# levayz/diffusion_finetuning

Measured on AMD Instinct MI355X. Metric: images/s SD1.5 LoRA rank-4 512^2 train step, higher is better.
Workload: dtype f16; 1 GPU; SD1.5 UNet-only LoRA rank=4, batch=4/GPU, 512^2 (64x64x4 latents), f16 storage/compute, fp32 accumulate + fp32 master LoRA, full train step (fwd+bwd+clip+AdamW); global_batch=4, parallelism=dp1, lora_params=1246464, overflow=False, hipgraph=True, conv_autotune=True, rccl_ranks=1

## Files before the change

diffusion_finetuning_amd/_native.py:

```python
import ctypes
import os
import threading

import torch

_LIB_PATH = os.environ.get("DFA_LIB_PATH") or os.path.join(os.path.dirname(os.path.abspath(__file__)), "lib", "liblora_hip.so")
_lib = None
_lock = threading.Lock()

ABI_VERSION = 9
PROF_KINDS = 18

_DTYPE_CODE = {torch.float32: 0, torch.float16: 1, torch.bfloat16: 2}

_vp, _i64, _i32, _f32 = ctypes.c_void_p, ctypes.c_int64, ctypes.c_int, ctypes.c_float


class GradProblem(ctypes.Structure):
    _fields_ = [
        ("S", _vp), ("P", _vp), ("out", _vp * 4),
        ("s_stride", _i64), ("p_stride", _i64), ("part_stride", _i64), ("M", _i64),
        ("C", _i32), ("r", _i32), ("rg", _i32), ("out_kn", _i32), ("n_blocks", _i32),
        ("scale", _f32),
    ]
# ... 76 lines not shown
                                            ctypes.c_uint64, _i32, _vp]),
    "ddpm_sample_step_keep_shared": (_i32, [_vp] * 11 + [_i32, _i64, _i64, _i32, _i32, _f32, _i32, _vp]),
    "ddpm_sample_multistep_keep_shared": (_i32, [_vp] * 13 + [_i32, _i64, _i64, _i32, _i32, _f32, _i32, _vp]),
    "ddpm_sample_sigma_init": (_i32, [_vp] * 7 + [_i32, _i64, _i32, _i32, _f32, _f32, _f32, _i32, _i32, ctypes.c_uint64, _i32, _vp]),
    "ddpm_sample_sigma": (_i32, [_vp] * 14 + [_i32, _i64, _i64, _i32, _i32, _i32, _f32, _i32, _vp]),
    "embed_rows_fwd": (_i32, [_vp, _vp, _vp, _i64, _i32, _i64, _i32, _vp]),
    "embed_rows_bwd": (_i32, [_vp, _vp, _vp, _vp, _i64, _i32, _i64, _i32, _i32, _vp]),
    "lora_adamw_rows": (_i32, [_vp, _vp, _vp, _vp, _vp, _i64, _i32, _vp, _f32, _f32, _f32, _f32, _f32, _f32, _f32, _i32, _vp]),
    "ti_rows_grad": (_i32, [_vp, _vp, _i64, _i32, _vp, _i32, _vp, _i32, _i32, _vp]),
    "ti_rows_adamw_decay": (_i32, [_vp, _i64, _i32, _vp, _i32, _vp, _vp, _vp, _f32, _f32, _f32, _f32, _f32, _f32, _i32, _f32, _f32,
                                   _vp]),
    "geglu_linear_bwd": (_i32, [_vp, _vp, _vp, _vp, _vp, _i64, _i32, _i32, _i32, _vp]),
    "geglu_gate_fwd": (_i32, [_vp, _vp, _i64, _i32, _i32, _vp]),
    "geglu_gate_bwd": (_i32, [_vp, _vp, _vp, _i64, _i32, _i32, _vp]),
    "attn_split_heads": (_i32, [_vp, _vp, _i32, _i32, _i32, _i32, _i32, _i32, _vp]),
    "attn_merge_heads": (_i32, [_vp, _vp, _i32, _i32, _i32, _i32, _i32, _i32, _vp]),
    "attn_merge_heads_strided": (_i32, [_vp, _vp, _i32, _i32, _i32, _i32, _i32, _i64, _i64, _i64, _i32, _vp]),
    "group_norm_act_workspace_bytes": (_i64, [_i32, _i32, _i32, _i32, _i32, _i32]),
    "group_norm_act_plan": (_i32, [_i32, _i32, _i32, _i32, _i32, _i32]),
    "group_norm_act_fwd": (_i32, [_vp] * 8 + [_i32, _i32, _i32, _i32, _f32, _i32, _i32, _i32, _vp]),
    "group_norm_act_bwd": (_i32, [_vp] * 10 + [_i32, _i32, _i32, _i32, _i32, _i32, _i32, _vp]),
    "group_norm_act_bwd_res": (_i32, [_vp] * 11 + [_i32, _i32, _i32, _i32, _i32, _i32, _vp]),
    "residual_bias_add_supported": (_i32, [_i32, _i32, _i32, _i32]),
    "residual_bias_add": (_i32, [_vp] * 5 + [_i32, _i32, _i32, _i32, _vp]),
    "tokens_nchw_supported": (_i32, [_i32, _i32, _i32, _i32]),
    "tokens_to_nchw_add": (_i32, [_vp] * 3 + [_i32, _i32, _i32, _i32, _vp]),
    "nchw_to_tokens": (_i32, [_vp] * 2 + [_i32, _i32, _i32, _i32, _vp]),
    "conv3x3_small_supported": (_i32, [_i32, _i32, _i32, _i32, _i32, _i32]),
    "conv3x3_small_workspace_bytes": (_i64, [_i32, _i32, _i32, _i32, _i32, _i32]),
    "conv3x3_small_plan": (_i32, [_i64, _i32, _i32, _i32]),
    "conv3x3_small_plan_channels": (_i32, [_i32, _i32, _i32]),
    "conv3x3_small_pack": (_i32, [_vp, _vp, _i32, _i32, _i32, _i32, _vp]),
    "conv3x3_small": (_i32, [_vp] * 5 + [_i64, _i32, _i32, _i32, _i32, _i32, _i32, _vp]),
    "add_layer_norm_max_channels": (_i32, []),
    "add_layer_norm_fwd": (_i32, [_vp] * 8 + [_i64, _i32, _f32, _i32, _vp]),
    "add_layer_norm_bwd": (_i32, [_vp] * 7 + [_i64, _i32, _i32, _vp]),
    "attn_ctx_supported": (_i32, [_i32, _i32, _i32, _i32, _i32, _i32]),
    "attn_ctx_fwd": (_i32, [_vp, _vp, _vp, _vp, _i32, _i32, _i32, _i32, _i32, _f32, _i32, _vp]),
    "attn_ctx_bwd_workspace_bytes": (_i64, [_i32, _i32, _i32, _i32, _i32]),
    "attn_ctx_fwd_strided": (_i32, [_vp, _vp, _vp, _vp, _i64, _i32, _i32, _i32, _i32, _i32, _f32, _i32, _vp]),
    "attn_ctx_bwd_strided": (_i32, [_vp] * 8 + [_i64, _i64, _i32, _i32, _i32, _i32, _i32, _f32, _i32, _vp]),
    "attn_flash_fwd_strided": (_i32, [_vp, _vp, _vp, _vp, _vp, _i64, _i32, _i32, _i32, _i32, _i32, _f32, _i32, _vp]),
    "attn_flash_bwd_strided": (_i32, [_vp] * 10 + [_i64, _i64, _i32, _i32, _i32, _i32, _i32, _f32, _i32, _vp]),
    "attn_ctx_bwd": (_i32, [_vp, _vp, _vp, _vp, _vp, _vp, _vp, _vp, _i32, _i32, _i32, _i32, _i32, _f32, _i32, _vp]),
    "attn_causal_supported": (_i32, [_i32, _i32, _i32, _i32, _i32]),
    "attn_causal_fwd_strided": (_i32, [_vp, _vp, _vp, _vp, _i64, _i32, _i32, _i32, _i32, _f32, _i32, _vp]),
    "attn_causal_bwd_workspace_bytes": (_i64, [_i32, _i32, _i32, _i32]),
    "attn_causal_bwd_strided": (_i32, [_vp] * 8 + [_i64, _i64, _i32, _i32, _i32, _i32, _f32, _i32, _vp]),
    "attn_flash_supported": (_i32, [_i32, _i32, _i32, _i32, _i32, _i32]),
    "attn_flash_fwd": (_i32, [_vp, _vp, _vp, _vp, _vp, _i32, _i32, _i32, _i32, _i32, _f32, _i32, _vp]),
    "attn_flash_bwd_workspace_bytes": (_i64, [_i32, _i32, _i32]),
    "attn_flash_bwd": (_i32, [_vp] * 10 + [_i32, _i32, _i32, _i32, _i32, _f32, _i32, _vp]),
    "attn_f32_supported": (_i32, [_i32, _i32, _i32, _i32, _i32]),
    "attn_f32_fwd": (_i32, [_vp, _vp, _vp, _vp, _vp, _i32, _i32, _i32, _i32, _i32, _f32, _vp]),
    "attn_f32_bwd_workspace_bytes": (_i64, [_i32, _i32, _i32]),
    "attn_f32_bwd": (_i32, [_vp] * 10 + [_i32, _i32, _i32, _i32, _i32, _f32, _vp]),
    "lora_distill_workspace_bytes": (_i64, [_i64, _i64]),
    "lora_distill_start": (_i32, [_vp, _i32, _i64, _i32, _i64, _vp, _vp]),
    "lora_distill_diff": (_i32, [_vp, _i32, _i64, _i32, _i32, _vp, _vp]),
    "lora_distill_rayleigh_ritz": (_i32, [_vp, _i32, _i32, _i32, ctypes.c_double, _i32, _vp, _vp]),
    "lora_distill_finalize": (_i32, [_vp, _i32, _i32, _f32, _i32, _vp, _vp, _vp]),
    "lora_quantile_clamp": (_i32, [_vp, _i64, _f32, _vp, _vp]),
    "lora_distill_wide_width": (_i32, [_i32]),
    "lora_distill_wide_workspace_bytes": (_i64, [_i64, _i64, _i32]),
    "lora_distill_wide_start": (_i32, [_vp, _i32, _i64, _i32, _i64, _vp, _vp]),
    "lora_distill_wide_diff": (_i32, [_vp, _i32, _i64, _i32, _i32, _i32, _vp, _vp]),
# ... 1112 lines not shown
def conv3x3_small_supported(N: int, Cin: int, Cout: int, H: int, W: int, dtype) -> bool:
    return dtype in (torch.float16, torch.bfloat16) and bool(lib().conv3x3_small_supported(N, Cin, Cout, H, W, dtype_code(dtype)))


def conv3x3_small_plan(pixels: int, Cin: int, Cout: int, dtype) -> bool:
    return dtype in (torch.float16, torch.bfloat16) and bool(lib().conv3x3_small_plan(int(pixels), Cin, Cout, dtype_code(dtype)))


def conv3x3_small_plan_channels(Cin: int, Cout: int, dtype) -> bool:
    return dtype in (torch.float16, torch.bfloat16) and bool(lib().conv3x3_small_plan_channels(Cin, Cout, dtype_code(dtype)))


def conv3x3_small_pack(weight, backward: bool):
    _require_device(weight)
    Cout, Cin = weight.shape[:2]
    packed = torch.empty(weight.numel(), dtype=weight.dtype, device=weight.device)
    _check(lib().conv3x3_small_pack(_ptr(weight), _ptr(packed), Cin, Cout, int(backward), dtype_code(weight.dtype),
                                    _stream(weight)), "conv3x3_small_pack")
    return packed


def conv3x3_small(x, pack, bias, Cout: int):
    _require_device(x, pack, bias)
    N, Cin, H, W = x.shape
    code = dtype_code(x.dtype)
    nbytes = int(lib().conv3x3_small_workspace_bytes(N, Cin, Cout, H, W, code))
    ws = torch.empty(max(nbytes, 16) // 4, dtype=torch.float32, device=x.device)
    y = torch.empty((N, Cout, H, W), dtype=x.dtype, device=x.device)
    _check(lib().conv3x3_small(_ptr(x), _ptr(pack), _ptr(bias), _ptr(y), _ptr(ws), nbytes, N, Cin, Cout, H, W, code, _stream(x)),
           "conv3x3_small")
    return y


def tokens_nchw_supported(N: int, C: int, HW: int, dtype) -> bool:
    return dtype in (torch.float16, torch.bfloat16) and bool(lib().tokens_nchw_supported(N, C, HW, dtype_code(dtype)))


def tokens_to_nchw_add(tok, res, shape):
    _require_device(tok, res)
    N, C, H, W = shape
    out = torch.empty(shape, dtype=tok.dtype, device=tok.device)
    _check(lib().tokens_to_nchw_add(_ptr(tok), _ptr(res), _ptr(out), N, C, H * W, dtype_code(tok.dtype), _stream(tok)),
           "tokens_to_nchw_add")
    return out


def nchw_to_tokens(x):
    _require_device(x)
    N, C, H, W = x.shape
    tok = torch.empty((N, H * W, C), dtype=x.dtype, device=x.device)
    _check(lib().nchw_to_tokens(_ptr(x), _ptr(tok), N, C, H * W, dtype_code(x.dtype), _stream(x)), "nchw_to_tokens")
    return tok


def add_layer_norm_supported(x) -> bool:
    C = x.shape[-1] if x.dim() else 0
    return (x.numel() > 0 and x.is_contiguous() and C % 8 == 0 and C <= lib().add_layer_norm_max_channels() and
            x.data_ptr() % 16 == 0)


def add_layer_norm_fwd(x, delta, gamma, beta, eps: float):
    _require_device(x, delta, gamma, beta)
    C = x.shape[-1]
    M = x.numel() // C
    h = None if delta is None else torch.empty_like(x)
    y = torch.empty_like(x)
# ... 262 lines not shown
```

diffusion_finetuning_amd/build_native.py:

```python
import hashlib
import os
import subprocess
import sys
from concurrent.futures import ThreadPoolExecutor

PKG_DIR = os.path.dirname(os.path.abspath(__file__))
CSRC = os.path.join(PKG_DIR, "csrc")
LIB_DIR = os.path.join(PKG_DIR, "lib")
LIB_PATH = os.path.join(LIB_DIR, "liblora_hip.so")
SOURCES = ["lora_gemm.hip", "lora_grad.hip", "ddpm_loss.hip", "optim.hip", "sandwich.hip", "norm.hip", "trunk_edges.hip", "conv_small.hip", "layer_norm.hip", "attn_ctx.hip", "attn_causal.hip", "attn_flash.hip", "attn_f32.hip", "embed.hip", "distill.hip", "distill_wide.hip", "prof.hip"]
HIPCC = os.environ.get("HIPCC", "/opt/rocm/bin/hipcc")
FLAGS = ["--offload-arch=gfx950", "-O3", "-std=c++17", "-fPIC", "-Wall", "-Wno-unused-function"]
SOURCE_FLAGS = {}


def _digest() -> str:
    h = hashlib.sha256()
    for name in sorted(os.listdir(CSRC)) + [os.path.join("..", "..", "include", "lora_hip.h")]:
        with open(os.path.join(CSRC, name), "rb") as f:
            h.update(name.encode())
            h.update(f.read())
    h.update(" ".join(FLAGS).encode())
    for name in sorted(SOURCE_FLAGS):
        h.update((name + " " + " ".join(SOURCE_FLAGS[name])).encode())
    return h.hexdigest()


def build(force: bool = False, verbose: bool = True, variant: str = "", defines=()) -> str:
    os.makedirs(LIB_DIR, exist_ok=True)
    lib_path = os.path.join(LIB_DIR, f"liblora_hip_{variant}.so") if variant else LIB_PATH
    obj_dir = os.path.join(LIB_DIR, f"obj_{variant}") if variant else LIB_DIR
    os.makedirs(obj_dir, exist_ok=True)
    stamp = os.path.join(LIB_DIR, f"liblora_hip_{variant}.stamp" if variant else "liblora_hip.stamp")
    digest = _digest() + (" " + " ".join(defines) if defines else "")
    if not force and os.path.exists(lib_path) and os.path.exists(stamp):
        with open(stamp) as f:
            if f.read().strip() == digest:
                return lib_path

    def compile_one(src: str) -> str:
        obj = os.path.join(obj_dir, src.replace(".hip", ".o"))
        cmd = [HIPCC, *FLAGS, *SOURCE_FLAGS.get(src, []), *defines, "-c", os.path.join(CSRC, src), "-o", obj]
        if verbose:
# ... 24 lines not shown
```

diffusion_finetuning_amd/conv.py:

```python
import torch
import torch.nn as nn
import torch.nn.functional as F
from torch.autograd.function import once_differentiable
from torch.utils.weak import WeakIdKeyDictionary

from . import _native as nat

ROUTES = ("auto", "hip", "stock")

_packs = WeakIdKeyDictionary()


def _key(weight):
    return (weight.data_ptr(), weight._version, weight.dtype, weight.device)


def _get_packs(weight):
    entry = _packs.get(weight)
    key = _key(weight)
    if entry is not None and entry[0] == key:
        return entry[1], entry[2]
    if torch.cuda.is_current_stream_capturing():
        return None
    w = weight.detach()
    entry = (key, nat.conv3x3_small_pack(w, False), nat.conv3x3_small_pack(w, True))
    _packs[weight] = entry
    return entry[1], entry[2]


def _weight_eligible(weight, bias) -> bool:
    if not weight.is_cuda or weight.dtype not in (torch.float16, torch.bfloat16) or weight.dim() != 4:
        return False
    if tuple(weight.shape[2:]) != (3, 3) or weight.shape[0] % 32 or weight.shape[1] % 32 or not weight.is_contiguous():
        return False
    if weight.data_ptr() % 16 or weight.requires_grad:
        return False
    if bias is not None and (bias.requires_grad or bias.dtype != weight.dtype or bias.device != weight.device or
                             bias.shape != weight.shape[:1] or not bias.is_contiguous()):
        return False
    return True


def _supported(x, weight, bias) -> bool:
    if not _weight_eligible(weight, bias):
        return False
    if x.dim() != 4 or x.dtype != weight.dtype or x.device != weight.device or x.shape[1] != weight.shape[1]:
        return False
    if x.numel() == 0 or not x.is_contiguous() or x.data_ptr() % 16:
        return False
    N, Cin, H, W = x.shape
    Cout = weight.shape[0]
    return nat.conv3x3_small_supported(N, Cin, Cout, H, W, x.dtype) and nat.conv3x3_small_supported(N, Cout, Cin, H, W, x.dtype)


class _Conv3x3Fn(torch.autograd.Function):
    @staticmethod
    def forward(ctx, x, weight, bias, fwd_pack, bwd_pack):
        ctx.bwd_pack = bwd_pack
        ctx.cin = x.shape[1]
        return nat.conv3x3_small(x, fwd_pack, bias, weight.shape[0])

    @staticmethod
    @once_differentiable
    def backward(ctx, dy):
        if not ctx.needs_input_grad[0]:
            return None, None, None, None, None
        dy = dy.contiguous()
        if dy.data_ptr() % 16:
            dy = dy.clone()
        return nat.conv3x3_small(dy, ctx.bwd_pack, None, ctx.cin), None, None, None, None


def conv3x3(x: torch.Tensor, weight: torch.Tensor, bias=None, route: str = "auto") -> torch.Tensor:
    if route not in ROUTES:
        raise ValueError(f"conv3x3: route must be one of {ROUTES}, got {route!r}")
    if route != "stock":
        ok = _supported(x, weight, bias)
        if ok and route == "auto":
            N, Cin, H, W = x.shape
            ok = nat.conv3x3_small_plan(N * H * W, Cin, weight.shape[0], x.dtype)
        packs = _get_packs(weight) if ok else None
        if packs is not None:
            return _Conv3x3Fn.apply(x, weight, bias, packs[0], packs[1])
        if route == "hip":
            raise RuntimeError("conv3x3(route='hip'): the HIP kernel does not cover this call (needs a frozen 16-bit 3×3 weight "
                               "with channel counts that are multiples of 32, an NCHW-contiguous x of the same dtype from a "
                               "16-byte boundary, and a pack made before stream capture)")
    return F.conv2d(x, weight, bias, padding=1)


def prepack_conv3x3(module: nn.Module, route: str = "auto") -> int:
    if route not in ROUTES:
        raise ValueError(f"prepack_conv3x3: route must be one of {ROUTES}, got {route!r}")
    if route == "stock":
        return 0
    n = 0
    for m in module.modules():
        if type(m) is not nn.Conv2d or m.kernel_size != (3, 3) or m.stride != (1, 1) or m.padding != (1, 1):
            continue
        if m.dilation != (1, 1) or m.groups != 1 or not _weight_eligible(m.weight, m.bias):
            continue
        if route == "auto" and not nat.conv3x3_small_plan_channels(m.weight.shape[1], m.weight.shape[0], m.weight.dtype):
            continue
        if _get_packs(m.weight) is not None:
            n += 1
    return n


def packed_bytes() -> int:
    return sum(e[1].numel() * e[1].element_size() + e[2].numel() * e[2].element_size() for e in _packs.values())
```

diffusion_finetuning_amd/csrc/conv_small.hip:

```cpp
#include "common.h"

namespace {

constexpr int kThreads = 256;
constexpr int kNT = 128;
constexpr int kChunk = 32;
constexpr int kPitch = 80;
constexpr int kCUs = 256;

template <typename T> struct Mfma;
template <> struct Mfma<half_t> {
    using Frag = f16x8;
    static __device__ __forceinline__ f32x4 run(Frag a, Frag b, f32x4 c) {
        return __builtin_amdgcn_mfma_f32_16x16x32_f16(a, b, c, 0, 0, 0);
    }
};
template <> struct Mfma<bf16_t> {
    using Frag = bf16x8;
    static __device__ __forceinline__ f32x4 run(Frag a, Frag b, f32x4 c) {
        return __builtin_amdgcn_mfma_f32_16x16x32_bf16(a, b, c, 0, 0, 0);
    }
};

__host__ __device__ __forceinline__ int padded_pos(int m, int H, int W) {
    const int HW = H * W, img = m / HW, r = m - img * HW, h = r / W, w = r - h * W;
    return img * (H + 2) * (W + 2) + (h + 1) * (W + 2) + (w + 1);
}
__host__ __device__ __forceinline__ int tile_positions(int m0, int MT, int M, int H, int W) {
    const int mlast = (m0 + MT < M ? m0 + MT : M) - 1;
    return padded_pos(mlast, H, W) - padded_pos(m0, H, W) + 2 * (W + 3) + 1;
}

__device__ __forceinline__ int fast_div(int n, int d, float inv) {
    int q = (int)((float)n * inv);
    int r = n - q * d;
    q += r >= d ? 1 : 0;
    q -= r < 0 ? 1 : 0;
    return q;
}

template <typename T, int MT, int PER>
__global__ __launch_bounds__(kThreads) void conv_small_kernel(const T* __restrict__ x, const T* __restrict__ wp,
                                                              float* __restrict__ part, int Cin, int Cout, int H, int W, int M,
                                                              int mtiles, int ntiles, int cps, int chunks, int Mpad) {
    using Frag = typename Mfma<T>::Frag;
    constexpr int MF = MT / 32;
    extern __shared__ __attribute__((aligned(16))) unsigned char smem[];
    const int tid = threadIdx.x, lane = tid & 63, wave = tid >> 6, wm = wave & 1, wn = wave >> 1;

    int mt, nt, sl;
    {
        const unsigned total = gridDim.x, id = blockIdx.x;
        const unsigned q = total >> 3, rem = total & 7, xcd = id & 7, slot = id >> 3;
        const unsigned n = (xcd < rem ? xcd * (q + 1) : rem * (q + 1) + (xcd - rem) * q) + slot;
        mt = (int)(n % (unsigned)mtiles);
        const unsigned rest = n / (unsigned)mtiles;
        nt = (int)(rest % (unsigned)ntiles);
        sl = (int)(rest / (unsigned)ntiles);
    }
    const int c_begin = sl * cps, c_end = min(c_begin + cps, chunks);
    const int HW = H * W, W2 = W + 2, PP = (H + 2) * W2;
    const int m0 = mt * MT;
    const int q0 = padded_pos(m0, H, W);
    const int P = tile_positions(m0, MT, M, H, W);
    const int qlo = q0 - (W2 + 1);
    const float inv_pp = 1.f / (float)PP, inv_w2 = 1.f / (float)W2;

    int xoff[PER];
    bool in_tile[PER];
#pragma unroll
    for (int s = 0; s < PER; ++s) {
        const int p = tid + s * kThreads;
// ... 120 lines not shown
        struct alignas(8) Out4 { T v[4]; } o;
#pragma unroll
        for (int i = 0; i < 4; ++i) o.v[i] = from_f32<T>(v[i] + b);
        *reinterpret_cast<Out4*>(dst) = o;
    } else {
        dst[0] = from_f32<T>(v[0] + b);
    }
}

template <typename T>
__global__ __launch_bounds__(256) void conv_small_pack_kernel(const T* __restrict__ w, T* __restrict__ out, int Cin, int Cout,
                                                              int backward) {
    const int64_t total = (int64_t)Cin * Cout * 9, o = (int64_t)blockIdx.x * 256 + threadIdx.x;
    if (o >= total) return;
    const int Co = backward ? Cin : Cout, KO = Co >> 4;
    const int j = (int)(o & 7), l = (int)((o >> 3) & 63);
    const int64_t rest = o >> 9;
    const int ko = (int)(rest % KO);
    const int64_t rest2 = rest / KO;
    const int t = (int)(rest2 % 9), cc = (int)(rest2 / 9);
    const int ci = cc * 32 + (l >> 4) * 8 + j, co = ko * 16 + (l & 15);
    const int64_t src = backward ? ((int64_t)ci * Cin + co) * 9 + (8 - t) : ((int64_t)co * Cin + ci) * 9 + t;
    out[o] = w[src];
}

struct Geo {
    int MT = 0, per = 0, mtiles = 0, ntiles = 0, chunks = 0, cps = 0, S = 0, Pcap = 0, Mpad = 0, M = 0;
    int64_t ws_bytes = 0;
    bool ok = false;
};

Geo conv_geo(int N, int Cin, int Cout, int H, int W) {
    Geo g;
    if (N < 1 || H < 1 || W < 1 || Cin < 32 || Cout < 32 || Cin % 32 || Cout % 32) return g;
    const int64_t M64 = (int64_t)N * H * W;
    if (M64 > (1 << 22) || M64 * Cin >= (1ll << 31) || M64 * Cout >= (1ll << 31) || (int64_t)(H + 2) * (W + 2) * N >= (1ll << 22))
        return g;
    const int M = (int)M64;
    const int mts[2] = {128, 64}, per[2] = {1, 3};
    for (int v = 0; v < 2 && !g.ok; ++v) {
        const int MT = mts[v], mtiles = (M + MT - 1) / MT;
        int pmax = 0;
        for (int t = 0; t < mtiles; ++t) {
            const int p = tile_positions(t * MT, MT, M, H, W);
            pmax = p > pmax ? p : pmax;
        }
        if (pmax > per[v] * kThreads) continue;
        g.MT = MT, g.per = per[v], g.mtiles = mtiles, g.Pcap = pmax, g.ok = true;
    }
    if (!g.ok) return g;
    g.M = M;
    g.Mpad = g.mtiles * g.MT;
    g.ntiles = (Cout + kNT - 1) / kNT;
    g.chunks = Cin / kChunk;
    const int tiles = g.mtiles * g.ntiles, want = kCUs / tiles > 1 ? kCUs / tiles : 1;
    int cps = (g.chunks + want - 1) / want;
    if (g.chunks >= 4 && cps < 2) cps = 2;
    g.cps = cps;
    g.S = (g.chunks + cps - 1) / cps;
    g.ws_bytes = (int64_t)g.S * Cout * g.Mpad * 4;
    if ((int64_t)tiles * g.S > (1 << 20)) g.ok = false;
    return g;
}

template <typename T, int MT, int PER>
bool launch_main(const T* x, const T* wp, float* part, int Cin, int Cout, int H, int W, const Geo& g, hipStream_t s) {
    const int lds = g.Pcap * kPitch;
    auto kern = conv_small_kernel<T, MT, PER>;
    if (lds > 48 * 1024 &&
        hipFuncSetAttribute(reinterpret_cast<const void*>(kern), hipFuncAttributeMaxDynamicSharedMemorySize, lds) != hipSuccess)
        return false;
// ... 89 lines not shown
```

include/lora_hip.h:

```cpp
#ifndef LORA_HIP_H
#define LORA_HIP_H

#include <stdint.h>

#ifdef __cplusplus
extern "C" {
#endif

#define LORA_HIP_ABI_VERSION 9

enum lora_dtype { LORA_F32 = 0, LORA_F16 = 1, LORA_BF16 = 2 };

enum lora_status {
    LORA_OK = 0,
    LORA_E_BADARG = -1,
    LORA_E_RANK = -2,
    LORA_E_ALIGN = -3,
    LORA_E_LAUNCH = -4,
    LORA_E_UNSUPPORTED = -5
};

int lora_version(void);

const char* lora_status_string(int status);
// ... 191 lines not shown
int attn_merge_heads(const void* src, void* dst, int B, int N, int H, int d, int D, int dtype, void* stream);
int attn_merge_heads_strided(const void* src, void* dst, int B, int N, int H, int d, int D, int64_t sB, int64_t sH,
                             int64_t sN, int dtype, void* stream);

int64_t group_norm_act_workspace_bytes(int N, int C, int HW, int groups, int channels_last, int want_da);
int group_norm_act_plan(int N, int C, int HW, int groups, int channels_last, int backward);
int group_norm_act_fwd(const void* x, const void* addend , const void* gamma, const void* beta, void* y,
                       float* mean, float* rstd, void* workspace, int N, int C, int HW, int groups, float eps, int act,
                       int channels_last, int dtype, void* stream);
int group_norm_act_bwd(const void* dy, const void* x, const void* addend , const void* gamma, const void* beta,
                       const float* mean, const float* rstd, void* dx, void* da , void* workspace, int N, int C,
                       int HW, int groups, int act, int channels_last, int dtype, void* stream);
int group_norm_act_bwd_res(const void* dy, const void* dh , const void* x, const void* addend ,
                           const void* gamma, const void* beta, const float* mean, const float* rstd, void* dx,
                           void* da , void* workspace, int N, int C, int HW, int groups, int act, int dtype,
                           void* stream);

int residual_bias_add_supported(int N, int C, int HW, int dtype);
int residual_bias_add(const void* h, const void* res, const void* b1, const void* b2 , void* out, int N, int C,
                      int HW, int dtype, void* stream);
int tokens_nchw_supported(int N, int C, int HW, int dtype);
int tokens_to_nchw_add(const void* tok, const void* res , void* out, int N, int C, int HW, int dtype,
                       void* stream);
int nchw_to_tokens(const void* x, void* tok, int N, int C, int HW, int dtype, void* stream);

int conv3x3_small_supported(int N, int C_in, int C_out, int H, int W, int dtype);
int64_t conv3x3_small_workspace_bytes(int N, int C_in, int C_out, int H, int W, int dtype);
int conv3x3_small_plan(int64_t pixels, int C_in, int C_out, int dtype);
int conv3x3_small_plan_channels(int C_in, int C_out, int dtype);
int conv3x3_small_pack(const void* w, void* packed, int C_in, int C_out, int backward, int dtype, void* stream);
int conv3x3_small(const void* x, const void* wpack, const void* bias , void* y, void* workspace,
                  int64_t workspace_bytes, int N, int C_in, int C_out, int H, int W, int dtype, void* stream);

int add_layer_norm_max_channels(void);
int add_layer_norm_fwd(const void* x, const void* delta , const void* gamma, const void* beta,
                       void* h , void* y, float* mean, float* rstd, int64_t M, int C, float eps,
                       int dtype, void* stream);
int add_layer_norm_bwd(const void* dy, const void* dh , const void* h, const void* gamma, const float* mean,
                       const float* rstd, void* dx, int64_t M, int C, int dtype, void* stream);

int embed_rows_fwd(const float* table, const int64_t* ids, void* out, int64_t n, int D, int64_t V, int out_dtype, void* stream);
int embed_rows_bwd(const void* dE, const int64_t* ids, float* grad_table, unsigned char* active , int64_t n,
                   int D, int64_t V, int dtype, int accumulate, void* stream);
int lora_adamw_rows(float* param, const float* grad, float* exp_avg, float* exp_avg_sq, const unsigned char* active, int64_t V,
                    int D, const float* norm_in, float grad_mul, float max_norm, float lr, float beta1, float beta2, float eps,
                    float weight_decay, int step, void* stream);

#define LORA_TI_MAX_ROWS 64
int ti_rows_grad(const void* dE, const int64_t* ids, int64_t n, int D, const int64_t* slot_ids, int P, float* grad, int dtype,
                 int accumulate, void* stream);
int ti_rows_adamw_decay(float* table, int64_t V, int D, const int64_t* slot_ids, int P, const float* grad, float* exp_avg,
                        float* exp_avg_sq, float grad_mul, float lr, float beta1, float beta2, float eps, float weight_decay,
                        int step, float decay_lambda, float target_norm, void* stream);

int attn_ctx_supported(int B, int Tq, int Tk, int H, int d, int dtype);
int attn_ctx_fwd_strided(const void* Q, const void* K, const void* V, void* O, int64_t ldk, int B, int Tq, int Tk,
                         int H, int d, float scale, int dtype, void* stream);
int attn_ctx_bwd_strided(const void* Q, const void* K, const void* V, const void* dO, void* dQ, void* dK, void* dV,
                         void* workspace, int64_t ldk, int64_t ld_dk, int B, int Tq, int Tk, int H, int d,
                         float scale, int dtype, void* stream);
int attn_ctx_fwd(const void* Q, const void* K, const void* V, void* O, int B, int Tq, int Tk, int H, int d,
                 float scale, int dtype, void* stream);
int64_t attn_ctx_bwd_workspace_bytes(int B, int Tq, int Tk, int H, int d);
int attn_ctx_bwd(const void* Q, const void* K, const void* V, const void* dO, void* dQ, void* dK, void* dV,
                 void* workspace, int B, int Tq, int Tk, int H, int d, float scale, int dtype, void* stream);

// ... 67 lines not shown
```

Baseline: 183.6 images/s.

## Add large-tile MFMA 3x3 conv kernel for mid-size SD UNet convolutions

Adds a second implicit-GEMM 3x3 convolution kernel with 160-wide output-channel tiles, triple-buffered weight staging loaded directly into LDS via global_load_lds, and XCD-aware block swizzling. The auto route now falls back to this kernel for SD1.5 channel/pixel combinations (4096 and 16384 pixels) that the small-conv plan rejected, replacing the stock conv path for those layers in forward and input-gradient backward. The aim is to beat the library conv on these shapes, but it adds a hand-tuned whitelist tied to specific UNet shapes and higher LDS usage per block.

```diff
diff --git a/diffusion_finetuning_amd/_native.py b/diffusion_finetuning_amd/_native.py
--- a/diffusion_finetuning_amd/_native.py
+++ b/diffusion_finetuning_amd/_native.py
@@ -132,6 +132,11 @@
     "conv3x3_small_plan_channels": (_i32, [_i32, _i32, _i32]),
     "conv3x3_small_pack": (_i32, [_vp, _vp, _i32, _i32, _i32, _i32, _vp]),
     "conv3x3_small": (_i32, [_vp] * 5 + [_i64, _i32, _i32, _i32, _i32, _i32, _i32, _vp]),
+    "conv3x3_large_supported": (_i32, [_i32, _i32, _i32, _i32, _i32, _i32]),
+    "conv3x3_large_workspace_bytes": (_i64, [_i32, _i32, _i32, _i32, _i32, _i32]),
+    "conv3x3_large_plan": (_i32, [_i64, _i32, _i32, _i32]),
+    "conv3x3_large_plan_channels": (_i32, [_i32, _i32, _i32]),
+    "conv3x3_large": (_i32, [_vp] * 5 + [_i64, _i32, _i32, _i32, _i32, _i32, _i32, _vp]),
     "add_layer_norm_max_channels": (_i32, []),
     "add_layer_norm_fwd": (_i32, [_vp] * 8 + [_i64, _i32, _f32, _i32, _vp]),
     "add_layer_norm_bwd": (_i32, [_vp] * 7 + [_i64, _i32, _i32, _vp]),
@@ -1310,6 +1315,27 @@
     return y
 
 
+def conv3x3_large_supported(N: int, Cin: int, Cout: int, H: int, W: int, dtype) -> bool:
+    return dtype in (torch.float16, torch.bfloat16) and bool(lib().conv3x3_large_supported(N, Cin, Cout, H, W, dtype_code(dtype)))
+
+
+def conv3x3_large_plan(pixels: int, Cin: int, Cout: int, dtype) -> bool:
+    return dtype in (torch.float16, torch.bfloat16) and bool(lib().conv3x3_large_plan(int(pixels), Cin, Cout, dtype_code(dtype)))
+
+
+def conv3x3_large_plan_channels(Cin: int, Cout: int, dtype) -> bool:
+    return dtype in (torch.float16, torch.bfloat16) and bool(lib().conv3x3_large_plan_channels(Cin, Cout, dtype_code(dtype)))
+
+
+def conv3x3_large(x, pack, bias, Cout: int):
+    _require_device(x, pack, bias)
+    N, Cin, H, W = x.shape
+    y = torch.empty((N, Cout, H, W), dtype=x.dtype, device=x.device)
+    _check(lib().conv3x3_large(_ptr(x), _ptr(pack), _ptr(bias), _ptr(y), None, 0, N, Cin, Cout, H, W, dtype_code(x.dtype),
+                               _stream(x)), "conv3x3_large")
+    return y
+
+
 def tokens_nchw_supported(N: int, C: int, HW: int, dtype) -> bool:
     return dtype in (torch.float16, torch.bfloat16) and bool(lib().tokens_nchw_supported(N, C, HW, dtype_code(dtype)))
 
diff --git a/diffusion_finetuning_amd/build_native.py b/diffusion_finetuning_amd/build_native.py
--- a/diffusion_finetuning_amd/build_native.py
+++ b/diffusion_finetuning_amd/build_native.py
@@ -8,7 +8,7 @@
 CSRC = os.path.join(PKG_DIR, "csrc")
 LIB_DIR = os.path.join(PKG_DIR, "lib")
 LIB_PATH = os.path.join(LIB_DIR, "liblora_hip.so")
-SOURCES = ["lora_gemm.hip", "lora_grad.hip", "ddpm_loss.hip", "optim.hip", "sandwich.hip", "norm.hip", "trunk_edges.hip", "conv_small.hip", "layer_norm.hip", "attn_ctx.hip", "attn_causal.hip", "attn_flash.hip", "attn_f32.hip", "embed.hip", "distill.hip", "distill_wide.hip", "prof.hip"]
+SOURCES = ["lora_gemm.hip", "lora_grad.hip", "ddpm_loss.hip", "optim.hip", "sandwich.hip", "norm.hip", "trunk_edges.hip", "conv_small.hip", "conv_large.hip", "layer_norm.hip", "attn_ctx.hip", "attn_causal.hip", "attn_flash.hip", "attn_f32.hip", "embed.hip", "distill.hip", "distill_wide.hip", "prof.hip"]
 HIPCC = os.environ.get("HIPCC", "/opt/rocm/bin/hipcc")
 FLAGS = ["--offload-arch=gfx950", "-O3", "-std=c++17", "-fPIC", "-Wall", "-Wno-unused-function"]
 SOURCE_FLAGS = {}
diff --git a/diffusion_finetuning_amd/conv.py b/diffusion_finetuning_amd/conv.py
--- a/diffusion_finetuning_amd/conv.py
+++ b/diffusion_finetuning_amd/conv.py
@@ -6,7 +6,9 @@
 
 from . import _native as nat
 
-ROUTES = ("auto", "hip", "stock")
+ROUTES = ("auto", "hip", "large", "stock")
+
+_FAMILY = {"hip": "small", "large": "large"}
 
 _packs = WeakIdKeyDictionary()
 
@@ -41,7 +43,7 @@
     return True
 
 
-def _supported(x, weight, bias) -> bool:
+def _supported(x, weight, bias, family="small") -> bool:
     if not _weight_eligible(weight, bias):
         return False
     if x.dim() != 4 or x.dtype != weight.dtype or x.device != weight.device or x.shape[1] != weight.shape[1]:
@@ -50,42 +52,62 @@
         return False
     N, Cin, H, W = x.shape
     Cout = weight.shape[0]
-    return nat.conv3x3_small_supported(N, Cin, Cout, H, W, x.dtype) and nat.conv3x3_small_supported(N, Cout, Cin, H, W, x.dtype)
+    covers = nat.conv3x3_small_supported if family == "small" else nat.conv3x3_large_supported
+    return covers(N, Cin, Cout, H, W, x.dtype) and covers(N, Cout, Cin, H, W, x.dtype)
+
+
+def _run(family, x, pack, bias, Cout):
+    return (nat.conv3x3_small if family == "small" else nat.conv3x3_large)(x, pack, bias, Cout)
+
+
+def _auto_family(pixels, Cin, Cout, dtype):
+    if nat.conv3x3_small_plan(pixels, Cin, Cout, dtype):
+        return "small"
+    if nat.conv3x3_large_plan(pixels, Cin, Cout, dtype):
+        return "large"
+    return None
 
 
 class _Conv3x3Fn(torch.autograd.Function):
     @staticmethod
-    def forward(ctx, x, weight, bias, fwd_pack, bwd_pack):
+    def forward(ctx, x, weight, bias, fwd_pack, bwd_pack, fwd_family, bwd_family):
         ctx.bwd_pack = bwd_pack
+        ctx.bwd_family = bwd_family
         ctx.cin = x.shape[1]
-        return nat.conv3x3_small(x, fwd_pack, bias, weight.shape[0])
+        return _run(fwd_family, x, fwd_pack, bias, weight.shape[0])
 
     @staticmethod
     @once_differentiable
     def backward(ctx, dy):
         if not ctx.needs_input_grad[0]:
-            return None, None, None, None, None
+            return (None,) * 7
         dy = dy.contiguous()
         if dy.data_ptr() % 16:
             dy = dy.clone()
-        return nat.conv3x3_small(dy, ctx.bwd_pack, None, ctx.cin), None, None, None, None
+        return (_run(ctx.bwd_family, dy, ctx.bwd_pack, None, ctx.cin),) + (None,) * 6
 
 
 def conv3x3(x: torch.Tensor, weight: torch.Tensor, bias=None, route: str = "auto") -> torch.Tensor:
     if route not in ROUTES:
         raise ValueError(f"conv3x3: route must be one of {ROUTES}, got {route!r}")
     if route != "stock":
-        ok = _supported(x, weight, bias)
-        if ok and route == "auto":
-            N, Cin, H, W = x.shape
-            ok = nat.conv3x3_small_plan(N * H * W, Cin, weight.shape[0], x.dtype)
-        packs = _get_packs(weight) if ok else None
+        fwd = bwd = None
+        if route == "auto":
+            if x.dim() == 4 and weight.dim() == 4 and x.is_cuda:
+                N, Cin, H, W = x.shape
+                fwd = _auto_family(N * H * W, Cin, weight.shape[0], x.dtype)
+                bwd = _auto_family(N * H * W, weight.shape[0], Cin, x.dtype) if fwd is not None else None
+                if bwd is None or not all(_supported(x, weight, bias, f) for f in {fwd, bwd}):
+                    fwd = bwd = None
+        elif _supported(x, weight, bias, _FAMILY[route]):
+            fwd = bwd = _FAMILY[route]
+        packs = _get_packs(weight) if fwd is not None else None
         if packs is not None:
-            return _Conv3x3Fn.apply(x, weight, bias, packs[0], packs[1])
-        if route == "hip":
-            raise RuntimeError("conv3x3(route='hip'): the HIP kernel does not cover this call (needs a frozen 16-bit 3×3 weight "
-                               "with channel counts that are multiples of 32, an NCHW-contiguous x of the same dtype from a "
-                               "16-byte boundary, and a pack made before stream capture)")
+            return _Conv3x3Fn.apply(x, weight, bias, packs[0], packs[1], fwd, bwd)
+        if route != "auto":
+            raise RuntimeError(f"conv3x3(route={route!r}): the HIP kernel does not cover this call (needs a frozen 16-bit 3×3 "
+                               "weight with channel counts that are multiples of 32, an NCHW-contiguous x of the same dtype "
+                               "from a 16-byte boundary, and a pack made before stream capture)")
     return F.conv2d(x, weight, bias, padding=1)
 
 
@@ -100,7 +122,8 @@
             continue
         if m.dilation != (1, 1) or m.groups != 1 or not _weight_eligible(m.weight, m.bias):
             continue
-        if route == "auto" and not nat.conv3x3_small_plan_channels(m.weight.shape[1], m.weight.shape[0], m.weight.dtype):
+        if route == "auto" and not (nat.conv3x3_small_plan_channels(m.weight.shape[1], m.weight.shape[0], m.weight.dtype) or
+                                    nat.conv3x3_large_plan_channels(m.weight.shape[1], m.weight.shape[0], m.weight.dtype)):
             continue
         if _get_packs(m.weight) is not None:
             n += 1
diff --git a/diffusion_finetuning_amd/csrc/conv_common.h b/diffusion_finetuning_amd/csrc/conv_common.h
--- /dev/null
+++ b/diffusion_finetuning_amd/csrc/conv_common.h
@@ -0,0 +1,48 @@
+#pragma once
+#include "common.h"
+
+namespace {
+
+constexpr int kThreads = 256;
+constexpr int kChunk = 32;
+constexpr int kPitch = 80;
+constexpr int kCUs = 256;
+
+template <typename T> struct Mfma;
+template <> struct Mfma<half_t> {
+    using Frag = f16x8;
+    static __device__ __forceinline__ f32x4 run(Frag a, Frag b, f32x4 c) {
+        return __builtin_amdgcn_mfma_f32_16x16x32_f16(a, b, c, 0, 0, 0);
+    }
+};
+template <> struct Mfma<bf16_t> {
+    using Frag = bf16x8;
+    static __device__ __forceinline__ f32x4 run(Frag a, Frag b, f32x4 c) {
+        return __builtin_amdgcn_mfma_f32_16x16x32_bf16(a, b, c, 0, 0, 0);
+    }
+};
+
+__host__ __device__ __forceinline__ int padded_pos(int m, int H, int W) {
+    const int HW = H * W, img = m / HW, r = m - img * HW, h = r / W, w = r - h * W;
+    return img * (H + 2) * (W + 2) + (h + 1) * (W + 2) + (w + 1);
+}
+__host__ __device__ __forceinline__ int tile_positions(int m0, int MT, int M, int H, int W) {
+    const int mlast = (m0 + MT < M ? m0 + MT : M) - 1;
+    return padded_pos(mlast, H, W) - padded_pos(m0, H, W) + 2 * (W + 3) + 1;
+}
+
+__device__ __forceinline__ int fast_div(int n, int d, float inv) {
+    int q = (int)((float)n * inv);
+    int r = n - q * d;
+    q += r >= d ? 1 : 0;
+    q -= r < 0 ? 1 : 0;
+    return q;
+}
+
+inline bool conv_shape_in_range(int N, int Cin, int Cout, int H, int W) {
+    if (N < 1 || H < 1 || W < 1 || Cin < 32 || Cout < 32 || Cin % 32 || Cout % 32) return false;
+    const int64_t M64 = (int64_t)N * H * W;
+    return !(M64 > (1 << 22) || M64 * Cin >= (1ll << 31) || M64 * Cout >= (1ll << 31) || (int64_t)(H + 2) * (W + 2) * N >= (1ll << 22));
+}
+
+}
diff --git a/diffusion_finetuning_amd/csrc/conv_large.hip b/diffusion_finetuning_amd/csrc/conv_large.hip
--- /dev/null
+++ b/diffusion_finetuning_amd/csrc/conv_large.hip
@@ -0,0 +1,300 @@
+#include <atomic>
+
+#include "conv_common.h"
+
+namespace {
+
+constexpr int kNTL = 160;
+constexpr int kFragsN = kNTL / 16;
+constexpr int kGroupFrags = 3 * kFragsN;
+constexpr int kWBuf = kGroupFrags * 1024;
+constexpr int kWBufs = 3;
+constexpr int kPieceSlots = 32;
+
+template <int N> __device__ __forceinline__ void wait_barrier() {
+    asm volatile("s_waitcnt vmcnt(%0) lgkmcnt(0)\n\ts_barrier" ::"n"(N) : "memory");
+}
+
+__device__ __forceinline__ void glds16(const void* gsrc, unsigned char* lds_wave_base) {
+    __builtin_amdgcn_global_load_lds((const __attribute__((address_space(1))) void*)(gsrc),
+                                     (__attribute__((address_space(3))) void*)(lds_wave_base), 16, 0, 0);
+}
+
+template <typename T, int MT, int PER, int WM>
+__global__ __launch_bounds__(WM * 128) void conv_large_kernel(const T* __restrict__ x, const T* __restrict__ wp,
+                                                              const T* __restrict__ bias, T* __restrict__ y, int Cin, int Cout,
+                                                              int H, int W, int M, int mtiles, int chunks, int Pcap) {
+    using Frag = typename Mfma<T>::Frag;
+    constexpr int NTHR = WM * 128, NW = WM * 2, kPieces = kPieceSlots / NW;
+    constexpr int MF = MT / (16 * WM);
+    constexpr int NF = kFragsN / 2;
+    extern __shared__ __attribute__((aligned(1024))) unsigned char smem[];
+    unsigned char* const wlds = smem;
+    unsigned char* const alds = smem + kWBufs * kWBuf;
+    const int abytes = Pcap * kPitch;
+    const int tid = threadIdx.x, lane = tid & 63, wave = __builtin_amdgcn_readfirstlane(tid >> 6), wm = wave % WM, wn = wave / WM;
+
+    int mt, nt;
+    {
+        const unsigned total = gridDim.x, id = blockIdx.x;
+        const unsigned q = total >> 3, rem = total & 7, xcd = id & 7, slot = id >> 3;
+        const unsigned n = (xcd < rem ? xcd * (q + 1) : rem * (q + 1) + (xcd - rem) * q) + slot;
+        mt = (int)(n % (unsigned)mtiles);
+        nt = (int)(n / (unsigned)mtiles);
+    }
+    const int HW = H * W, W2 = W + 2, PP = (H + 2) * W2;
+    const int m0 = mt * MT;
+    const int q0 = padded_pos(m0, H, W);
+    const int P = tile_positions(m0, MT, M, H, W);
+    const int qlo = q0 - (W2 + 1);
+    const float inv_pp = 1.f / (float)PP, inv_w2 = 1.f / (float)W2, inv_p = 1.f / (float)P;
+
+    int xoff[PER];
+    int aoff[PER];
+#pragma unroll
+    for (int s = 0; s < PER; ++s) {
+        const int i = tid + s * NTHR, cg = fast_div(i, P, inv_p), p = i - cg * P;
+        const bool unit = cg < 4;
+        const int q = qlo + p, img = fast_div(q, PP, inv_pp), r = q - img * PP, hp = fast_div(r, W2, inv_w2), wq = r - hp * W2;
+        const bool inside = unit && hp >= 1 && hp <= H && wq >= 1 && wq <= W;
+        xoff[s] = inside ? (img * Cin + cg * 8) * HW + (hp - 1) * W + (wq - 1) : -1;
+        aoff[s] = unit ? p * kPitch + cg * 16 : 2 * abytes + tid * 16;
+    }
+    T raw[PER][8];
+    auto load_stage = [&](int cc) {
+        const T* base = x + (size_t)cc * kChunk * HW;
+#pragma unroll
+        for (int s = 0; s < PER; ++s) {
+            const int o = xoff[s] >= 0 ? xoff[s] : 0;
+#pragma unroll
+            for (int c = 0; c < 8; ++c) raw[s][c] = base[o + c * HW];
+        }
+    };
+    auto write_stage = [&](int buf) {
+#pragma unroll
+        for (int s = 0; s < PER; ++s) {
+            Frag v;
+#pragma unroll
+            for (int j = 0; j < 8; ++j) v[j] = xoff[s] >= 0 ? raw[s][j] : static_cast<T>(0.f);
+            *reinterpret_cast<Frag*>(alds + (aoff[s] < 2 * abytes ? buf * abytes : 0) + aoff[s]) = v;
+        }
+    };
+
+    int lpos[MF];
+    const float inv_hw = 1.f / (float)HW, inv_w = 1.f / (float)W;
+#pragma unroll
+    for (int f = 0; f < MF; ++f) {
+        const int m = min(m0 + wm * (MT / WM) + f * 16 + (lane & 15), M - 1);
+        const int img = fast_div(m, HW, inv_hw), r = m - img * HW, h = fast_div(r, W, inv_w);
+        lpos[f] = (img * PP + (h + 1) * W2 + (r - h * W) + 1 - q0) * kPitch + (lane >> 4) * 16;
+    }
+
+    const int KO = Cout >> 4;
+    const size_t tap_stride = (size_t)KO * 512;
+    const int c0 = mt % chunks;
+    auto chunk_of = [&](int it) { const int c = c0 + it; return c >= chunks ? c - chunks : c; };
+    auto load_w = [&](int st, int slot, int lo, int hi) {
+        const T* src = wp + (size_t)(chunk_of(st / 3) * 3 + st % 3) * 3 * tap_stride + lane * 8;
+        unsigned char* dst = wlds + slot * kWBuf;
+#pragma unroll
+        for (int i = lo; i < hi; ++i) {
+            const int j = min(wave + NW * i, kGroupFrags - 1), t = j / kFragsN, f = j - t * kFragsN;
+            glds16(src + t * tap_stride + (size_t)min(nt * kFragsN + f, KO - 1) * 512, dst + j * 1024);
+        }
+    };
+
+    f32x4 acc[MF][NF];
+#pragma unroll
+    for (int f = 0; f < MF; ++f)
+#pragma unroll
+        for (int g = 0; g < NF; ++g) acc[f][g] = f32x4{0.f, 0.f, 0.f, 0.f};
+
+    static_assert(kPieces + 8 * PER <= 63, "vmcnt is a 6-bit counter");
+    constexpr int kP1 = (kPieces * 3 + 7) / 8 + (kPieces < 8), kP2 = kP1 + (kPieces - kP1 + 1) / 2;
+    const int steps = chunks * 3;
+    load_stage(c0);
+    load_w(0, 0, 0, kPieces);
+    load_w(min(1, steps - 1), 1, 0, kPieces);
+    write_stage(0);
+    for (int cc = 0; cc < chunks; ++cc) {
+        const unsigned char* ab = alds + (cc & 1) * abytes;
+#pragma unroll
+        for (int r = 0; r < 3; ++r) {
+            const int st = cc * 3 + r, ahead = min(st + 2, steps - 1), aslot = (r + 2) % 3;
+            if (r == 1) wait_barrier<kPieces + 8 * PER>();
+            else wait_barrier<kPieces>();
+            if (r == 2) write_stage((cc + 1) & 1);
+            load_w(ahead, aslot, 0, kP1);
+            if (r == 0) load_stage(chunk_of(min(cc + 1, chunks - 1)));
+            __builtin_amdgcn_sched_barrier(0);
+            const unsigned char* wb = wlds + r * kWBuf + wn * NF * 1024 + lane * 16;
+            Frag xf[2][MF], bf[2][NF];
+            {
+                const int sh = (r * W2) * kPitch;
+#pragma unroll
+                for (int f = 0; f < MF; ++f) xf[0][f] = *reinterpret_cast<const Frag*>(ab + lpos[f] + sh);
+#pragma unroll
+                for (int g = 0; g < NF; ++g) bf[0][g] = *reinterpret_cast<const Frag*>(wb + g * 1024);
+            }
+#pragma unroll
+            for (int tt = 0; tt < 3; ++tt) {
+                if (tt + 1 < 3) {
+                    const int sh = (r * W2 + tt + 1) * kPitch;
+#pragma unroll
+                    for (int f = 0; f < MF; ++f) xf[(tt + 1) & 1][f] = *reinterpret_cast<const Frag*>(ab + lpos[f] + sh);
+#pragma unroll
+                    for (int g = 0; g < NF; ++g)
+                        bf[(tt + 1) & 1][g] = *reinterpret_cast<const Frag*>(wb + ((tt + 1) * kFragsN + g) * 1024);
+                }
+#pragma unroll
+                for (int f = 0; f < MF; ++f)
+#pragma unroll
+                    for (int g = 0; g < NF; ++g) acc[f][g] = Mfma<T>::run(xf[tt & 1][f], bf[tt & 1][g], acc[f][g]);
+                if (tt < 2) load_w(ahead, aslot, tt == 0 ? kP1 : kP2, tt == 0 ? kP2 : kPieces);
+                __builtin_amdgcn_sched_barrier(0);
+            }
+        }
+    }
+
+    asm volatile("s_waitcnt vmcnt(0)" ::: "memory");
+
+    const bool quad = (HW & 3) == 0;
+    struct alignas(8) Out4 { T v[4]; };
+#pragma unroll
+    for (int g = 0; g < NF; ++g) {
+        const int k = nt * kNTL + (wn * NF + g) * 16 + (lane & 15);
+        if (k >= Cout) continue;
+        const float b = bias ? to_f32(bias[k]) : 0.f;
+#pragma unroll
+        for (int f = 0; f < MF; ++f) {
+            const int m = m0 + wm * (MT / WM) + f * 16 + (lane >> 4) * 4;
+            if (quad) {
+                if (m < M) {
+                    const int img = fast_div(m, HW, inv_hw);
+                    Out4 o;
+#pragma unroll
+                    for (int i = 0; i < 4; ++i) o.v[i] = from_f32<T>(acc[f][g][i] + b);
+                    *reinterpret_cast<Out4*>(y + (img * Cout + k) * HW + (m - img * HW)) = o;
+                }
+            } else {
+#pragma unroll
+                for (int i = 0; i < 4; ++i)
+                    if (m + i < M) {
+                        const int img = fast_div(m + i, HW, inv_hw);
+                        y[(img * Cout + k) * HW + (m + i - img * HW)] = from_f32<T>(acc[f][g][i] + b);
+                    }
+            }
+        }
+    }
+}
+
+struct LGeo {
+    int MT = 0, per = 0, mtiles = 0, ntiles = 0, chunks = 0, Pcap = 0, M = 0;
+    bool ok = false;
+};
+
+constexpr int kVariants = 3;
+constexpr int kVarMT[kVariants] = {128, 64, 64};
+constexpr int kVarPer[kVariants] = {3, 3, 6};
+constexpr int kVarWM[kVariants] = {4, 2, 2};
+
+int max_positions(int MT, int M, int H, int W) {
+    const int HW = H * W, mtiles = (M + MT - 1) / MT;
+    int a = MT, b = HW;
+    while (b) { const int c = a % b; a = b, b = c; }
+    const int period = HW / a;
+    int pmax = 0;
+    for (int t = 0; t < mtiles && t < period; ++t) {
+        const int p = tile_positions(t * MT, MT, M, H, W);
+        pmax = p > pmax ? p : pmax;
+    }
+    return pmax;
+}
+
+LGeo large_geo(int N, int Cin, int Cout, int H, int W) {
+    LGeo g;
+    if (!conv_shape_in_range(N, Cin, Cout, H, W)) return g;
+    const int M = N * H * W, ntiles = (Cout + kNTL - 1) / kNTL;
+    const int p128 = max_positions(128, M, H, W), p64 = max_positions(64, M, H, W);
+    const bool fits[kVariants] = {p128 <= 32 * kVarWM[0] * kVarPer[0], p64 <= 32 * kVarWM[1] * kVarPer[1],
+                                  p64 <= 32 * kVarWM[2] * kVarPer[2]};
+    int v = -1;
+    if (fits[0] && (int64_t)((M + 127) / 128) * ntiles >= kCUs) v = 0;
+    else if (fits[1]) v = 1;
+    else if (fits[2]) v = 2;
+    if (v < 0) return g;
+    g.MT = kVarMT[v], g.per = kVarPer[v], g.Pcap = v == 0 ? p128 : p64;
+    g.mtiles = (M + g.MT - 1) / g.MT, g.ntiles = ntiles, g.chunks = Cin / kChunk, g.M = M;
+    g.ok = (int64_t)g.mtiles * g.ntiles <= (1 << 20);
+    return g;
+}
+
+template <typename T, int MT, int PER, int WM>
+bool launch_large(const T* x, const T* wp, const T* bias, T* y, int Cin, int Cout, int H, int W, const LGeo& g, hipStream_t s) {
+    const int lds = kWBufs * kWBuf + 2 * g.Pcap * kPitch + WM * 128 * 16;
+    auto kern = conv_large_kernel<T, MT, PER, WM>;
+    static std::atomic<int> lds_allowed{0};
+    if (lds > lds_allowed.load(std::memory_order_relaxed)) {
+        if (hipFuncSetAttribute(reinterpret_cast<const void*>(kern), hipFuncAttributeMaxDynamicSharedMemorySize, lds) != hipSuccess)
+            return false;
+        lds_allowed.store(lds, std::memory_order_relaxed);
+    }
+    hipLaunchKernelGGL(kern, dim3(g.mtiles * g.ntiles), dim3(WM * 128), lds, s, x, wp, bias, y, Cin, Cout, H, W, g.M, g.mtiles,
+                       g.chunks, g.Pcap);
+    return true;
+}
+
+template <typename T>
+int run_large(const void* x_, const void* wp_, const void* bias_, void* y_, int Cin, int Cout, int H, int W, const LGeo& g,
+              hipStream_t s) {
+    const T *x = static_cast<const T*>(x_), *wp = static_cast<const T*>(wp_), *bias = static_cast<const T*>(bias_);
+    T* y = static_cast<T*>(y_);
+    const bool ok = g.MT == 128   ? launch_large<T, 128, 3, 4>(x, wp, bias, y, Cin, Cout, H, W, g, s)
+                    : g.per == 3 ? launch_large<T, 64, 3, 2>(x, wp, bias, y, Cin, Cout, H, W, g, s)
+                                 : launch_large<T, 64, 6, 2>(x, wp, bias, y, Cin, Cout, H, W, g, s);
+    if (!ok) return LORA_E_LAUNCH;
+    LORA_LAUNCH_CHECK();
+    return LORA_OK;
+}
+
+bool large_plan_channels(int C_in, int C_out, int64_t pixels ) {
+    const int lo = C_in < C_out ? C_in : C_out, hi = C_in < C_out ? C_out : C_in;
+    const bool at4096 = (lo == 640 && (hi == 640 || hi == 960 || hi == 1280 || hi == 1920)) || (lo == 320 && hi == 640) ||
+                        (lo == 1280 && hi == 1280);
+    const bool at16384 = (lo == 320 && (hi == 320 || hi == 640 || hi == 960)) || (lo == 640 && hi == 640);
+    return pixels == 4096 ? at4096 : pixels == 16384 ? at16384 : pixels == 0 ? (at4096 || at16384) : false;
+}
+
+}
+
+extern "C" int conv3x3_large_supported(int N, int C_in, int C_out, int H, int W, int dtype) {
+    return (dtype == LORA_F16 || dtype == LORA_BF16) && large_geo(N, C_in, C_out, H, W).ok ? 1 : 0;
+}
+
+extern "C" int64_t conv3x3_large_workspace_bytes(int N, int C_in, int C_out, int H, int W, int dtype) {
+    (void)N, (void)C_in, (void)C_out, (void)H, (void)W, (void)dtype;
+    return 0;
+}
+
+extern "C" int conv3x3_large_plan(int64_t pixels, int C_in, int C_out, int dtype) {
+    if (dtype != LORA_F16 && dtype != LORA_BF16) return 0;
+    return pixels >= 1 && large_plan_channels(C_in, C_out, pixels) ? 1 : 0;
+}
+
+extern "C" int conv3x3_large_plan_channels(int C_in, int C_out, int dtype) {
+    if (dtype != LORA_F16 && dtype != LORA_BF16) return 0;
+    return large_plan_channels(C_in, C_out, 0) ? 1 : 0;
+}
+
+extern "C" int conv3x3_large(const void* x, const void* wpack, const void* bias, void* y, void* workspace, int64_t workspace_bytes,
+                             int N, int C_in, int C_out, int H, int W, int dtype, void* stream) {
+    if (!x || !wpack || !y || N < 1 || C_in < 1 || C_out < 1 || H < 1 || W < 1) return LORA_E_BADARG;
+    if (dtype != LORA_F16 && dtype != LORA_BF16) return dtype == LORA_F32 ? LORA_E_UNSUPPORTED : LORA_E_BADARG;
+    const LGeo g = large_geo(N, C_in, C_out, H, W);
+    if (!g.ok) return LORA_E_UNSUPPORTED;
+    if (workspace_bytes < 0) return LORA_E_BADARG;
+    if (!aligned16(x) || !aligned16(wpack) || !aligned16(y) || !aligned16(workspace)) return LORA_E_ALIGN;
+    hipStream_t s = static_cast<hipStream_t>(stream);
+    return dtype == LORA_F16 ? run_large<half_t>(x, wpack, bias, y, C_in, C_out, H, W, g, s)
+                             : run_large<bf16_t>(x, wpack, bias, y, C_in, C_out, H, W, g, s);
+}
diff --git a/diffusion_finetuning_amd/csrc/conv_small.hip b/diffusion_finetuning_amd/csrc/conv_small.hip
--- a/diffusion_finetuning_amd/csrc/conv_small.hip
+++ b/diffusion_finetuning_amd/csrc/conv_small.hip
@@ -1,43 +1,8 @@
-#include "common.h"
+#include "conv_common.h"
 
 namespace {
 
-constexpr int kThreads = 256;
 constexpr int kNT = 128;
-constexpr int kChunk = 32;
-constexpr int kPitch = 80;
-constexpr int kCUs = 256;
-
-template <typename T> struct Mfma;
-template <> struct Mfma<half_t> {
-    using Frag = f16x8;
-    static __device__ __forceinline__ f32x4 run(Frag a, Frag b, f32x4 c) {
-        return __builtin_amdgcn_mfma_f32_16x16x32_f16(a, b, c, 0, 0, 0);
-    }
-};
-template <> struct Mfma<bf16_t> {
-    using Frag = bf16x8;
-    static __device__ __forceinline__ f32x4 run(Frag a, Frag b, f32x4 c) {
-        return __builtin_amdgcn_mfma_f32_16x16x32_bf16(a, b, c, 0, 0, 0);
-    }
-};
-
-__host__ __device__ __forceinline__ int padded_pos(int m, int H, int W) {
-    const int HW = H * W, img = m / HW, r = m - img * HW, h = r / W, w = r - h * W;
-    return img * (H + 2) * (W + 2) + (h + 1) * (W + 2) + (w + 1);
-}
-__host__ __device__ __forceinline__ int tile_positions(int m0, int MT, int M, int H, int W) {
-    const int mlast = (m0 + MT < M ? m0 + MT : M) - 1;
-    return padded_pos(mlast, H, W) - padded_pos(m0, H, W) + 2 * (W + 3) + 1;
-}
-
-__device__ __forceinline__ int fast_div(int n, int d, float inv) {
-    int q = (int)((float)n * inv);
-    int r = n - q * d;
-    q += r >= d ? 1 : 0;
-    q -= r < 0 ? 1 : 0;
-    return q;
-}
 
 template <typename T, int MT, int PER>
 __global__ __launch_bounds__(kThreads) void conv_small_kernel(const T* __restrict__ x, const T* __restrict__ wp,
@@ -224,11 +189,8 @@
 
 Geo conv_geo(int N, int Cin, int Cout, int H, int W) {
     Geo g;
-    if (N < 1 || H < 1 || W < 1 || Cin < 32 || Cout < 32 || Cin % 32 || Cout % 32) return g;
-    const int64_t M64 = (int64_t)N * H * W;
-    if (M64 > (1 << 22) || M64 * Cin >= (1ll << 31) || M64 * Cout >= (1ll << 31) || (int64_t)(H + 2) * (W + 2) * N >= (1ll << 22))
-        return g;
-    const int M = (int)M64;
+    if (!conv_shape_in_range(N, Cin, Cout, H, W)) return g;
+    const int M = N * H * W;
     const int mts[2] = {128, 64}, per[2] = {1, 3};
     for (int v = 0; v < 2 && !g.ok; ++v) {
         const int MT = mts[v], mtiles = (M + MT - 1) / MT;
diff --git a/include/lora_hip.h b/include/lora_hip.h
--- a/include/lora_hip.h
+++ b/include/lora_hip.h
@@ -247,6 +247,13 @@
 int conv3x3_small(const void* x, const void* wpack, const void* bias , void* y, void* workspace,
                   int64_t workspace_bytes, int N, int C_in, int C_out, int H, int W, int dtype, void* stream);
 
+int conv3x3_large_supported(int N, int C_in, int C_out, int H, int W, int dtype);
+int64_t conv3x3_large_workspace_bytes(int N, int C_in, int C_out, int H, int W, int dtype);
+int conv3x3_large_plan(int64_t pixels, int C_in, int C_out, int dtype);
+int conv3x3_large_plan_channels(int C_in, int C_out, int dtype);
+int conv3x3_large(const void* x, const void* wpack, const void* bias , void* y, void* workspace ,
+                  int64_t workspace_bytes, int N, int C_in, int C_out, int H, int W, int dtype, void* stream);
+
 int add_layer_norm_max_channels(void);
 int add_layer_norm_fwd(const void* x, const void* delta , const void* gamma, const void* beta,
                        void* h , void* y, float* mean, float* rstd, int64_t M, int C, float eps,
```

New measurement: 202.8 images/s (median of 6 runs). 10.5% higher.
